# mmp/pbrt-v1

Measured on AMD Instinct MI355X. Metric: Mrays/s (primary+secondary: every Scene::Intersect + Scene::IntersectP), higher is better.
Workload: dtype f32

## Files before the change

### pbrt-v1_amd/csrc/hip/rt_device.h

```cpp
#pragma once
#include "rt_math.h"
#include "../../../include/pbrt_hip.h"
#include "../../../include/pbrt_hip_texture.h"

namespace rt {

struct DevTri { float4 q0, q1, q2; };
#define RT_PRIM_QUADRIC (1u << 17)
struct DevQuadric {
    float w2o[16], o2w[16];
    float radius, zmin, zmax, theta_min, theta_max, phi_max;
    int type, pad;
    float p1[3], p2[3], a, c;
};

#define RT_PRIM_SHADING (1u << 18)
#define RT_PRIM_TEXTURED (1u << 19)
struct DevTriShading {
    unsigned flags, xform;
    float uv[6];
    float dpdu[3];
    float n[9], s[9];
    float pad[3];
};

typedef RtMaterialResolved DevMaterial;
struct DevMatTex { RtMaterialParams raw; int textured; int prog_off[RT_MATSLOT_COUNT], prog_len[RT_MATSLOT_COUNT]; };

struct DevLight {
    int type;
    float color[3];
    float pos[3];
    int n_samples;
    unsigned first_tri, n_tris;
    int reverse_orientation, flip_normal;
    float area;
    float dir[3];
    int quadric;
    float w2l[9];
    float cos_total, cos_falloff;
};

#define RT_MAX_DIM_REQ 12
struct DimReq { unsigned f_base, u_base; unsigned short n; unsigned short dims; };

struct DevScene {
    const DevTri *tris;
    const DevQuadric *quadrics;
    const float4 *tri_shade;
    const uint2 *nodes;
    const uint2 *tnodes;
    const uint4 *tpairs;
    unsigned root_x, root_y;
    unsigned top_pairs, leaf_runs;
// ... 2 lines not shown
    const unsigned *leaf_refs;
    const int *tri_shading_idx;
    const DevTriShading *tri_shading;
    const float *xforms;
    const DevMaterial *materials;
    const DevLight *lights;
    const float *light_tris;
    unsigned n_tris, n_lights;
    float bounds[6];
    int accel_kind;
    int nvox[3];
    float gwidth[3], ginv_width[3];
    RtCamera cam;
    RtVolume vol;
    int dens_kind;
    float dens_a, dens_b, dens_up[3];
    int dens_n[3];
    const float *dens_grid;
    int n_infinite;
    int n_textured;
    const RtTexture *tex_nodes;
    const int *tex_prog;
    const DevMatTex *mat_tex;
    const int *tex_uv_idx;
    const float *tex_uv;
};

#define RT_INTEG_DIRECT_WEIGHTED 3

struct DevFrame {
    int integrator, max_depth, strategy, volume_integrator;
    float step_size;
    int sampler, xs, ys, jitter, spp;
    unsigned seed;
    int x_pixel_start, y_pixel_start, x_pixel_count, y_pixel_count;
    int x_start, x_end, y_start, y_end;
    float fxw, fyw, inv_fxw, inv_fyw;
    const float *filter_table;
    float *accum;
    float4 *samples;
    int shard_index, shard_count, tile_pixels;
    int tile_w, tile_h, tiles_x;
    int dbg_x, dbg_y;
    int exit_thresh;
    int phase_sync;
    int high_occupancy;
    int leaf_min;
    int mega_tile;
    int xcd_bands;
    int trav_mode;
    int pipeline;
    unsigned long long total_work;
    unsigned long long total_pixels;
    int n1d, n2d;
    unsigned lhs_total;
    unsigned pixgen_draws;
    DimReq one_d[RT_MAX_DIM_REQ];
    DimReq two_d[RT_MAX_DIM_REQ];
    const DimReq *light_dims;
    int dims_max_n;
    unsigned long long *work_counter;
    unsigned long long *counters;
    uint2 *spill;
    float *frames;
    float *vol_rays, *vol_state, *vol_samp;
    int vol_nmax;
    unsigned n_threads;
    int weighted_phase;
    unsigned *wt_base;
    float *wt_rec;
    float2 *wt_pick;
    int wt_mixed;
    unsigned wt_nd;
    const unsigned *wt_recbase;
    unsigned mat_pool_base;
    int dens_cap;
#ifdef RT_TAIL_PROBE
    unsigned long long *probe;
#endif
};

#if defined(__HIP_DEVICE_COMPILE__)
#define RT_G __attribute__((address_space(1)))
#define RT_L __attribute__((address_space(3)))
#else
#define RT_G
#define RT_L
#endif
typedef const DevMaterial RT_G &MatRef;
typedef const DevLight RT_G &LightRef;
#define RT_MAT(sc, i) (*((const DevMaterial RT_G *)(sc).materials + (i)))
#define RT_LIGHT(sc, i) (*((const DevLight RT_G *)(sc).lights + (i)))
#define RT_GPTR(T, p) ((T RT_G *)(p))

#define RT_SAMPLE_XY 1
__host__ __device__ inline unsigned long long sample_slot(unsigned lp, unsigned s, int spp) {
    return ((unsigned long long)(lp >> 6) * unsigned(spp) + s) * 128ull + (lp & 63u) * 2u;
}

}
```

### pbrt-v1_amd/csrc/hip/rt_integrate.h

```cpp
#pragma once
#include "rt_shade.h"
#include "rt_texture.h"

namespace rt {

enum Stage {
    ST_FETCH = 0, ST_VERTEX, ST_DIRECT_NEXT, ST_SHADOW_DONE, ST_MIS_DONE, ST_ED_BSDF, ST_ED_DONE,
    ST_BOUNCE, ST_SPECULAR, ST_SPEC_TRANS, ST_RETURN, ST_VOL_BEGIN, ST_VOL_STEP, ST_POP, ST_FINISH, ST_EXIT
};

struct Rng {
    uint32_t base, ctr;
    RT_DEV float next_float() { return rng_f32(base, ctr++); }
    RT_DEV uint32_t next_u32() { return rng_u32(base, ctr++); }
};

#define RT_FRAME_WORDS 25

struct Lane {
    uint32_t sample_index;
    uint32_t work;
    float image_x, image_y;
    uint32_t dim_base;
    Rng rng;
// ... 32 lines not shown
        if (pos == k) pos = other; else if (pos == other) pos = k;
    }
    float delta = 1.f / n;
    return (pos + rng_f32(ln.rng.base, fb + pos * r.dims + d)) * delta;
}

RT_DEV float van_der_corput(uint32_t n, uint32_t scramble) {
    n = (n << 16) | (n >> 16);
    n = ((n & 0x00ff00ffu) << 8) | ((n & 0xff00ff00u) >> 8);
    n = ((n & 0x0f0f0f0fu) << 4) | ((n & 0xf0f0f0f0u) >> 4);
    n = ((n & 0x33333333u) << 2) | ((n & 0xccccccccu) >> 2);
    n = ((n & 0x55555555u) << 1) | ((n & 0xaaaaaaaau) >> 1);
    n ^= scramble;
    return (float)n / (float)0x100000000LL;
}
RT_DEV float sobol2(uint32_t n, uint32_t scramble) {
    for (uint32_t v = 1u << 31; n != 0; n >>= 1, v ^= v >> 1)
        if (n & 0x1) scramble ^= v;
    return (float)scramble / (float)0x100000000LL;
}
RT_DEV int shuffle_origin(uint32_t base, uint32_t off, int count, int pos) {
    for (int k = count - 1; k >= 0; --k) {
        const int other = int(rng_u32(base, off + k) % uint32_t(count));
        if (pos == k) pos = other; else if (pos == other) pos = k;
    }
    return pos;
}
RT_DEV uint32_t pixel_stream(const DevFrame &fr, const Lane &ln) {
    const uint32_t n0 = ln.sample_index - (ln.work % uint32_t(fr.spp));
    if (n0 == 0 && fr.sampler != RT_SAMPLER_LOWDISCREPANCY) return rng_base(0xFFFFFFFFu, fr.seed);
    return rng_base(n0, fr.seed);
}
RT_DEV float dim_value(const DevFrame &fr, const Lane &ln, const DimReq &r, int j, int d) {
    if (fr.sampler == RT_SAMPLER_STRATIFIED) return lhs_value(ln, r, j, d);
    if (fr.sampler == RT_SAMPLER_RANDOM) return rng_f32(ln.rng.base, ln.dim_base + r.f_base + j * r.dims + d);
    const uint32_t pb = pixel_stream(fr, ln);
    const int P = fr.spp, n = r.n, s = int(ln.work % uint32_t(P));
    const uint32_t nscr = r.dims;
    const int blk = shuffle_origin(pb, r.f_base + nscr + uint32_t(n) * P, P, s);
    const int jb = (n == 1) ? 0 : shuffle_origin(pb, r.f_base + nscr + uint32_t(blk) * n, n, j);
    const uint32_t idx = uint32_t(blk) * n + jb;
    if (r.dims == 1) return van_der_corput(idx, rng_u32(pb, r.f_base));
    return d == 0 ? van_der_corput(idx, rng_u32(pb, r.f_base)) : sobol2(idx, rng_u32(pb, r.f_base + 1));
}

#ifndef RT_SAMPLE_NT
#define RT_SAMPLE_NT 1
#endif
RT_DEV void sample_write(const DevFrame &fr, const Lane &ln, V3 Ls, float alpha, unsigned &bad) {
    const float y = lum_y(Ls);
    if (Ls.x != Ls.x || Ls.y != Ls.y || Ls.z != Ls.z) { Ls = mk3(0.f); ++bad; }
    else if (y < -1e-5) { Ls = mk3(0.f); ++bad; }
    else if (isinf(y)) { Ls = mk3(0.f); ++bad; }
    const uint32_t lp = ln.work / uint32_t(fr.spp);
    float4 RT_G *rec = RT_GPTR(float4, fr.samples) + sample_slot(lp, ln.work - lp * uint32_t(fr.spp), fr.spp);
#if RT_SAMPLE_NT
    typedef float nt_f4 __attribute__((ext_vector_type(4)));
    const nt_f4 r0 = {Ls.x, Ls.y, Ls.z, alpha}, r1 = {ln.image_x, ln.image_y, 0.f, 0.f};
    __builtin_nontemporal_store(r0, (nt_f4 RT_G *)rec);
    __builtin_nontemporal_store(r1, (nt_f4 RT_G *)(rec + RT_SAMPLE_XY));
#else
    rec[0] = make_float4(Ls.x, Ls.y, Ls.z, alpha);
    rec[RT_SAMPLE_XY] = make_float4(ln.image_x, ln.image_y, 0.f, 0.f);
#endif
}

RT_DEV void stratified_camera_sample(const DevFrame &fr, uint32_t pixel_index, int s, int px, int py,
                                     uint32_t pix_base, float &ix, float &iy, float &lu, float &lv, bool need_lens) {
    const int n = fr.spp;
    const int sx = s % fr.xs, sy = s / fr.xs;
    const float dx = 1.f / fr.xs, dy = 1.f / fr.ys;
    float jx = 0.5f, jy = 0.5f;
    if (fr.jitter) { jx = rng_f32(pix_base, 2 * s); jy = rng_f32(pix_base, 2 * s + 1); }
    ix = (sx + jx) * dx; iy = (sy + jy) * dy;
    ix += px; iy += py;
    lu = lv = 0.5f;
    if (need_lens) {
        const uint32_t ub = fr.jitter ? 5u * n : 0u;
        int pos = s;
        for (int k = n - 1; k >= 0; --k) {
            int other = int(rng_u32(pix_base, ub + k) % uint32_t(n));
            if (pos == k) pos = other; else if (pos == other) pos = k;
        }
        const int lx = pos % fr.xs, ly = pos / fr.xs;
        float kx = 0.5f, ky = 0.5f;
        if (fr.jitter) { kx = rng_f32(pix_base, 2 * n + 2 * pos); ky = rng_f32(pix_base, 2 * n + 2 * pos + 1); }
        lu = (lx + kx) * dx; lv = (ly + ky) * dy;
    }
    (void)pixel_index;
}

RT_DEV Ray camera_ray(const RtCamera &cam, float ix, float iy, float lensU, float lensV) {
    Ray r;
    if (cam.type == RT_CAMERA_ENVIRONMENT) {
        r.o = xform_point(cam.camera_to_world, mk3(0.f, 0.f, 0.f));
        const float theta = RT_PI * iy / cam.y_res;
        const float phi = 2 * RT_PI * ix / cam.x_res;
        const V3 dir = mk3(sinf(theta) * cosf(phi), cosf(theta), sinf(theta) * sinf(phi));
        r.d = xform_vector(cam.camera_to_world, dir);
        r.mint = cam.hither; r.maxt = cam.yon;
        return r;
    }
    V3 Pcamera = xform_point(cam.raster_to_camera, mk3(ix, iy, 0.f));
    r.o = Pcamera;
    r.d = cam.type == RT_CAMERA_ORTHOGRAPHIC ? mk3(0.f, 0.f, 1.f) : Pcamera;
    if (cam.lens_radius > 0.f) {
        float lu, lv; concentric_disk(lensU, lensV, lu, lv);
        lu *= cam.lens_radius; lv *= cam.lens_radius;
        float ft = (cam.focal_distance - cam.hither) / r.d.z;
        V3 Pfocus = r.o + r.d * ft;
        r.o.x += lu * (cam.focal_distance - cam.hither) / cam.focal_distance;
        r.o.y += lv * (cam.focal_distance - cam.hither) / cam.focal_distance;
        r.d = Pfocus - r.o;
    }
    r.d = normalize3(r.d);
    r.mint = 0.f;
    r.maxt = cam.type == RT_CAMERA_ORTHOGRAPHIC ? cam.yon - cam.hither : (cam.yon - cam.hither) / r.d.z;
    r.o = xform_point(cam.camera_to_world, r.o);
    r.d = xform_vector(cam.camera_to_world, r.d);
    return r;
}

RT_DEV bool work_to_sample(const DevFrame &fr, unsigned long long w, unsigned long long &pixel, int &s) {
    const unsigned long long per_tile = (unsigned long long)fr.tile_pixels * fr.spp;
    if (fr.tile_w > 0) {
        const unsigned w32 = unsigned(w), pt = unsigned(per_tile);
        const unsigned lt = w32 / pt, rem = w32 - lt * pt;
        const unsigned tile = lt * unsigned(fr.shard_count) + unsigned(fr.shard_index);
        const unsigned q = rem / unsigned(fr.spp);
        s = int(rem - q * unsigned(fr.spp));
        const unsigned ty = tile / unsigned(fr.tiles_x), tx = tile - ty * unsigned(fr.tiles_x);
        const unsigned qy = q / unsigned(fr.tile_w), qx = q - qy * unsigned(fr.tile_w);
        const unsigned px = tx * unsigned(fr.tile_w) + qx, py = ty * unsigned(fr.tile_h) + qy;
        const unsigned ew = unsigned(fr.x_end - fr.x_start), eh = unsigned(fr.y_end - fr.y_start);
        pixel = (unsigned long long)py * ew + px;
        return px < ew && py < eh;
    }
    if (fr.total_work <= 0xffffffffull && per_tile <= 0xffffffffull) {
        const unsigned w32 = unsigned(w), pt = unsigned(per_tile);
        const unsigned lt = w32 / pt, rem = w32 - lt * pt;
        const unsigned long long tile = (unsigned long long)lt * unsigned(fr.shard_count) + unsigned(fr.shard_index);
        const unsigned q = rem / unsigned(fr.spp);
        pixel = tile * unsigned(fr.tile_pixels) + q;
        s = int(rem - q * unsigned(fr.spp));
        return pixel < fr.total_pixels;
    }
    const unsigned long long lt = w / per_tile, rem = w % per_tile;
    const unsigned long long tile = lt * fr.shard_count + fr.shard_index;
    pixel = tile * fr.tile_pixels + rem / fr.spp;
    s = int(rem % fr.spp);
    return pixel < fr.total_pixels;
}

RT_DEV void tile_order_to_sample(const DevFrame &fr, unsigned w, unsigned &pixel, int &s) {
    const unsigned spp = unsigned(fr.spp), T = unsigned(fr.mega_tile);
    const unsigned W = unsigned(fr.x_end - fr.x_start), H = unsigned(fr.y_end - fr.y_start);
    const unsigned wp = w / spp; s = int(w - wp * spp);
    const unsigned row_px = W * T, ty = wp / row_px, rem = wp - ty * row_px;
    const unsigned h_t = min(T, H - ty * T), full = T * h_t, tiles_x = (W + T - 1u) / T;
    unsigned tx = rem / full; tx = tx < tiles_x ? tx : tiles_x - 1u;
    const unsigned rem2 = rem - tx * full, w_t = min(T, W - tx * T);
    const unsigned qy = rem2 / w_t, qx = rem2 - qy * w_t;
    pixel = (ty * T + qy) * W + tx * T + qx;
}

RT_DEV void setup_sample(const DevScene &sc, const DevFrame &fr, Lane &ln, unsigned long long pixel, int s, Ray &ray) {
    const int w = fr.x_end - fr.x_start;
    int px, py;
    if (fr.total_pixels <= 0xffffffffull) { const unsigned row = unsigned(pixel) / unsigned(w); px = fr.x_start + int(unsigned(pixel) - row * unsigned(w)); py = fr.y_start + int(row); }
    else { px = fr.x_start + int(pixel % w); py = fr.y_start + int(pixel / w); }
    const uint32_t n0 = uint32_t(pixel * fr.spp);
    ln.sample_index = n0 + uint32_t(s);
    ln.rng.base = rng_base(ln.sample_index, fr.seed);
    float lu = 0.5f, lv = 0.5f;
    const bool need_lens = sc.cam.lens_radius > 0.f;
    if (fr.sampler == RT_SAMPLER_STRATIFIED) {
        const uint32_t pix_base = (pixel == 0) ? rng_base(0xFFFFFFFFu, fr.seed) : rng_base(n0, fr.seed);
        ln.dim_base = (s == 0 && pixel != 0) ? fr.pixgen_draws : 0u;
        stratified_camera_sample(fr, uint32_t(pixel), s, px, py, pix_base, ln.image_x, ln.image_y, lu, lv, need_lens);
    } else if (fr.sampler == RT_SAMPLER_RANDOM) {
        const uint32_t pix_base = (pixel == 0) ? rng_base(0xFFFFFFFFu, fr.seed) : rng_base(n0, fr.seed);
        ln.dim_base = (s == 0 && pixel != 0) ? fr.pixgen_draws : 0u;
        ln.image_x = rng_f32(pix_base, 2 * s); ln.image_y = rng_f32(pix_base, 2 * s + 1);
        ln.image_x += px; ln.image_y += py;
        if (need_lens) { lu = rng_f32(pix_base, 2 * fr.spp + 2 * s); lv = rng_f32(pix_base, 2 * fr.spp + 2 * s + 1); }
    } else {
        const uint32_t pix_base = rng_base(n0, fr.seed);
        const uint32_t P = uint32_t(fr.spp);
        ln.dim_base = (s == 0) ? fr.pixgen_draws : 0u;
        const int pos = shuffle_origin(pix_base, 2 + P, int(P), s);
        ln.image_x = px + van_der_corput(uint32_t(pos), rng_u32(pix_base, 0));
        ln.image_y = py + sobol2(uint32_t(pos), rng_u32(pix_base, 1));
        if (need_lens) {
            const uint32_t lb = 2 + 2 * P;
            const int lp = shuffle_origin(pix_base, lb + 2 + P, int(P), s);
            lu = van_der_corput(uint32_t(lp), rng_u32(pix_base, lb)); lv = sobol2(uint32_t(lp), rng_u32(pix_base, lb + 1));
        }
    }
    ln.rng.ctr = ln.dim_base + ((fr.sampler == RT_SAMPLER_LOWDISCREPANCY) ? 0u : fr.lhs_total);
    ray = camera_ray(sc.cam, ln.image_x, ln.image_y, lu, lv);
    ln.image_x = (ln.image_x + 1.f) - 1.f; ln.image_y = (ln.image_y + 1.f) - 1.f;
}

RT_DEV float RT_G *frame_ptr(const DevFrame &fr, int frame, unsigned gtid) {
    return RT_GPTR(float, fr.frames) + (size_t(frame) * RT_FRAME_WORDS) * fr.n_threads + gtid;
}
template <bool EXT>
RT_DEV void frame_push(const DevFrame &fr, Lane &ln, unsigned gtid, V3 f, float absdot, int after) {
    float RT_G *q = frame_ptr(fr, ln.fsp, gtid); const size_t st = fr.n_threads;
    q[0 * st] = ln.L.x; q[1 * st] = ln.L.y; q[2 * st] = ln.L.z;
    q[3 * st] = f.x; q[4 * st] = f.y; q[5 * st] = f.z; q[6 * st] = absdot;
    q[7 * st] = __int_as_float(after); q[8 * st] = __int_as_float(ln.depth);
    q[9 * st] = ln.v.p.x; q[10 * st] = ln.v.p.y; q[11 * st] = ln.v.p.z;
    q[12 * st] = ln.v.nn.x; q[13 * st] = ln.v.nn.y; q[14 * st] = ln.v.nn.z;
    q[15 * st] = ln.v.sn.x; q[16 * st] = ln.v.sn.y; q[17 * st] = ln.v.sn.z;
    q[18 * st] = ln.v.wo.x; q[19 * st] = ln.v.wo.y; q[20 * st] = ln.v.wo.z;
    q[21 * st] = __int_as_float(ln.v.mat);
    if (EXT) { q[22 * st] = ln.v.ng.x; q[23 * st] = ln.v.ng.y; q[24 * st] = ln.v.ng.z; }
    ++ln.fsp;
}
template <bool EXT>
RT_DEV int frame_pop(const DevFrame &fr, Lane &ln, unsigned gtid, V3 child) {
    --ln.fsp;
    const float RT_G *q = frame_ptr(fr, ln.fsp, gtid); const size_t st = fr.n_threads;
    V3 Lp = mk3(q[0 * st], q[1 * st], q[2 * st]);
    V3 f = mk3(q[3 * st], q[4 * st], q[5 * st]);
    float absdot = q[6 * st];
    ln.L = Lp + (child * f) * absdot;
    int after = __float_as_int(q[7 * st]);
    ln.depth = __float_as_int(q[8 * st]);
    ln.v.p = mk3(q[9 * st], q[10 * st], q[11 * st]);
    ln.v.nn = mk3(q[12 * st], q[13 * st], q[14 * st]);
    ln.v.sn = mk3(q[15 * st], q[16 * st], q[17 * st]);
    ln.v.tn = cross3(ln.v.nn, ln.v.sn);
    ln.v.wo = mk3(q[18 * st], q[19 * st], q[20 * st]);
    ln.v.mat = __float_as_int(q[21 * st]);
    if (EXT) ln.v.ng = mk3(q[22 * st], q[23 * st], q[24 * st]);
    return after;
}

template <bool DEFER = false>
RT_DEV void launch_ray(Lane &ln, const DevScene &sc, V3 o, V3 d, float mint, float maxt, bool any, int next_stage) {
    Ray r; r.o = o; r.d = d; r.mint = mint; r.maxt = maxt;
    if (DEFER) { ln.tv.o = o; ln.tv.d = d; ln.tv.mint = mint; ln.tv.maxt = maxt; ln.tv.any = any; ln.tv.hit_prim = -1; ln.tv.b1 = 0.f; ln.tv.b2 = 0.f; }
    else if (sc.accel_kind == RT_ACCEL_GRID) grid_begin(ln.tv, sc, r, any); else trav_begin(ln.tv, sc, r, any);
    ln.has_ray = true;
    ln.stage = next_stage;
}

RT_DEV float RT_G *vol_ray_ptr(const DevFrame &fr, int level, unsigned gtid) { return RT_GPTR(float, fr.vol_rays) + size_t(level) * 8 * fr.n_threads + gtid; }
RT_DEV void vol_store_ray(const DevFrame &fr, int level, unsigned gtid, const Ray &r) {
    float RT_G *q = vol_ray_ptr(fr, level, gtid); const size_t st = fr.n_threads;
    q[0] = r.o.x; q[st] = r.o.y; q[2 * st] = r.o.z; q[3 * st] = r.d.x; q[4 * st] = r.d.y; q[5 * st] = r.d.z; q[6 * st] = r.mint; q[7 * st] = r.maxt;
}
RT_DEV Ray vol_load_ray(const DevFrame &fr, int level, unsigned gtid) {
    const float RT_G *q = vol_ray_ptr(fr, level, gtid); const size_t st = fr.n_threads;
    Ray r; r.o = mk3(q[0], q[st], q[2 * st]); r.d = mk3(q[3 * st], q[4 * st], q[5 * st]); r.mint = q[6 * st]; r.maxt = q[7 * st];
    return r;
}
RT_DEV bool vol_intersect(const RtVolume &v, V3 o, V3 d, float mint, float maxt, float &t0, float &t1) {
    const V3 vo = xform_point(v.world_to_volume, o), vd = xform_vector(v.world_to_volume, d);
    float a = mint, b = maxt; bool ok = true;
#pragma unroll
    for (int i = 0; i < 3; ++i) {
        float invRayDir = 1.f / comp(vd, i);
        float tNear = (v.p0[i] - comp(vo, i)) * invRayDir, tFar = (v.p1[i] - comp(vo, i)) * invRayDir;
        if (tNear > tFar) { float tmp = tNear; tNear = tFar; tFar = tmp; }
        a = tNear > a ? tNear : a; b = tFar < b ? tFar : b;
        if (a > b) ok = false;
    }
    t0 = a; t1 = b; return ok;
}
RT_DEV bool vol_inside(const RtVolume &v, V3 p) {
    const V3 q = xform_point(v.world_to_volume, p);
    return q.x >= v.p0[0] && q.x <= v.p1[0] && q.y >= v.p0[1] && q.y <= v.p1[1] && q.z >= v.p0[2] && q.z <= v.p1[2];
}
RT_DEV V3 vol_transmittance(const RtVolume &v, V3 o, V3 d, float mint, float maxt) {
    float t0, t1;
    if (!vol_intersect(v, o, d, mint, maxt, t0, t1)) return mk3(1.f);
    const float dist = len3((o + d * t0) - (o + d * t1));
    const V3 tau = (mat_color(v.sigma_a) + mat_color(v.sigma_s)) * dist;
    return mk3(expf(-tau.x), expf(-tau.y), expf(-tau.z));
}
RT_DEV float lerp_ref(float t, float v1, float v2) { return (1.f - t) * v1 + t * v2; }
RT_DEV int clamp_ref(int v, int lo, int hi) { return v < lo ? lo : (v > hi ? hi : v); }
RT_DEV float density_at(const DevScene &sc, V3 q) {
    const RtVolume &v = sc.vol;
    if (!(q.x >= v.p0[0] && q.x <= v.p1[0] && q.y >= v.p0[1] && q.y <= v.p1[1] && q.z >= v.p0[2] && q.z <= v.p1[2])) return 0.f;
    if (sc.dens_kind == RT_DENSITY_EXPONENTIAL) {
        const float height = (q.x - v.p0[0]) * sc.dens_up[0] + (q.y - v.p0[1]) * sc.dens_up[1] + (q.z - v.p0[2]) * sc.dens_up[2];
        return sc.dens_a * expf(-sc.dens_b * height);
// ... 316 lines not shown
        return;
    }
    if constexpr (STAGE == ST_DIRECT_NEXT) {
        const int nLights = int(sc.n_lights);
        if constexpr (WEIGHTED) {
            if (nLights == 0) { ln.stage = ST_SPECULAR; return; }
            if (fr.weighted_phase == 1) { ++ln.ord; ln.stage = ST_SPECULAR; return; }
            if (fr.weighted_phase == 3 && ln.li > 0) { ln.stage = ST_SPECULAR; return; }
            if (fr.weighted_phase == 2 && fr.wt_mixed) {
                if (ln.li == 0 && ln.lj == 0) { ln.ctr0 = ln.rng.ctr; ln.wt_w = __uint_as_float(1u); }
                if (ln.li >= nLights) { ++ln.ord; ln.rng.ctr = ln.ctr0; ln.lj = 0; ln.stage = ST_SPECULAR; return; }
                ln.rng.ctr = ln.ctr0 + uint32_t(ln.lj);
            } else if (fr.weighted_phase == 2) {
                if (ln.li == 0) ln.ctr0 = ln.rng.ctr;
                if (ln.li >= nLights) { ++ln.ord; ln.stage = ST_SPECULAR; return; }
                ln.rng.ctr = ln.ctr0;
            }
            const float ls1 = dim_value(fr, ln, fr.two_d[0], 0, 0), ls2 = dim_value(fr, ln, fr.two_d[0], 0, 1);
            ln.bs1 = dim_value(fr, ln, fr.two_d[1], 0, 0); ln.bs2 = dim_value(fr, ln, fr.two_d[1], 0, 1);
            ln.bcs = dim_value(fr, ln, fr.one_d[1], 0, 0);
            if (fr.weighted_phase == 2) {
                if (ln.li == 0 && ln.lj == 0) RT_GPTR(float, fr.wt_rec)[weighted_record(fr, ln, nLights)] = dim_value(fr, ln, fr.one_d[0], 0, 0);
                estimate_direct_begin<EXT, DEFER>(sc, ln, ln.li, ls1, ls2);
            } else {
                const float2 pick = RT_GPTR(const float2, fr.wt_pick)[ln.ord++];
                ln.li = 1; ln.wt_w = pick.y;
                estimate_direct_begin<EXT, DEFER>(sc, ln, __float_as_int(pick.x), ls1, ls2);
            }
            return;
        }
        if (INTEG == RT_INTEGRATOR_PATH || (INTEG == RT_INTEGRATOR_DIRECT && fr.strategy == RT_STRATEGY_ONE)) {
            if (nLights == 0 || ln.li > 0) { ln.stage = (INTEG == RT_INTEGRATOR_PATH) ? ST_BOUNCE : ST_SPECULAR; return; }
            ln.li = 1;
            const int k = (INTEG == RT_INTEGRATOR_PATH) ? ln.depth : 0;
            const bool from_sampler = (INTEG == RT_INTEGRATOR_DIRECT) || k < 3;
            float un, ls1, ls2;
            if (from_sampler) {
                const int i1 = (INTEG == RT_INTEGRATOR_PATH) ? 3 * k : 0;
                const int i2 = (INTEG == RT_INTEGRATOR_PATH) ? 3 * k : 0;
                un = dim_value(fr, ln, fr.one_d[i1], 0, 0);
                ls1 = dim_value(fr, ln, fr.two_d[i2], 0, 0); ls2 = dim_value(fr, ln, fr.two_d[i2], 0, 1);
                ln.bs1 = dim_value(fr, ln, fr.two_d[i2 + 1], 0, 0); ln.bs2 = dim_value(fr, ln, fr.two_d[i2 + 1], 0, 1);
                ln.bcs = dim_value(fr, ln, fr.one_d[i1 + 1], 0, 0);
            } else {
                un = ln.rng.next_float();
                ls1 = ln.rng.next_float(); ls2 = ln.rng.next_float();
                ln.bs1 = ln.rng.next_float(); ln.bs2 = ln.rng.next_float(); ln.bcs = ln.rng.next_float();
            }
            int lightNum = min(int(floorf(un * nLights)), nLights - 1);
            estimate_direct_begin<EXT, DEFER>(sc, ln, lightNum, ls1, ls2);
            return;
        }
        if (INTEG == RT_INTEGRATOR_DIRECT) {
            if (ln.li >= nLights) { ln.L = ln.L + ln.L_all; ln.stage = ST_SPECULAR; return; }
            const DimReq RT_G *ld = RT_GPTR(const DimReq, fr.light_dims) + 3 * ln.li;
            const DimReq rl = ld[0], rb = ld[1], rc = ld[2];
            if (ln.lj == 0) ln.Ld_light = mk3(0.f);
            const float ls1 = dim_value(fr, ln, rl, ln.lj, 0), ls2 = dim_value(fr, ln, rl, ln.lj, 1);
            ln.bs1 = dim_value(fr, ln, rb, ln.lj, 0); ln.bs2 = dim_value(fr, ln, rb, ln.lj, 1);
            ln.bcs = dim_value(fr, ln, rc, ln.lj, 0);
            estimate_direct_begin<EXT, DEFER>(sc, ln, ln.li, ls1, ls2);
            return;
        }
        if (ln.li >= nLights) { ln.stage = ST_SPECULAR; return; }
        {
            LightRef Lt = RT_LIGHT(sc, ln.li);
            MatRef m = RT_MAT(sc, ln.v.mat);
            const int cur = ln.li++;
            V3 wi, Li, sd; float smax;
            if (light_is_delta<EXT>(Lt)) Li = delta_light_sample(Lt, ln.v.p, wi, sd, smax);
            else if constexpr (EXT) {
                if (light_is_infinite<EXT>(Lt)) {
                    float u2 = ln.rng.next_float();
                    float u1 = ln.rng.next_float();
                    float pdf; wi = infinite_sample_sphere(u1, u2, pdf);
                    Li = (pdf == 0.f) ? mk3(0.f) : div_s(mat_color(Lt.color), pdf);
                    sd = wi; smax = RT_INF;
                } else {
                    float u2 = ln.rng.next_float();
                    float u1 = ln.rng.next_float();
                    V3 ns; V3 ps = area_sample_point<EXT>(sc, Lt, ln.v.p, u1, u2, ln.rng, ns);
                    wi = normalize3(ps - ln.v.p);
                    float pdf = area_light_pdf<EXT>(sc, Lt, ln.v.p, wi);
                    Li = (pdf == 0.f) ? mk3(0.f) : div_s(area_L(Lt, ns, -wi), pdf);
                    sd = ps - ln.v.p; smax = 1.f - RT_RAY_EPSILON;
                }
            } else {
                float u2 = ln.rng.next_float();
                float u1 = ln.rng.next_float();
                V3 ns; V3 ps = area_sample_point<EXT>(sc, Lt, ln.v.p, u1, u2, ln.rng, ns);
                wi = normalize3(ps - ln.v.p);
                float pdf = area_light_pdf<EXT>(sc, Lt, ln.v.p, wi);
                Li = (pdf == 0.f) ? mk3(0.f) : div_s(area_L(Lt, ns, -wi), pdf);
                sd = ps - ln.v.p; smax = 1.f - RT_RAY_EPSILON;
            }
            (void)cur;
            if (is_black(Li)) return;
            V3 f = bsdf_f<EXT>(m, ln.v, ln.v.wo, wi);
            if (is_black(f)) return;
            ln.pend = (f * Li) * absdot3(wi, ln.v.nn);
            launch_ray<DEFER>(ln, sc, ln.v.p, sd, RT_RAY_EPSILON, smax, true, ST_SHADOW_DONE);
        }
        return;
    }
    if constexpr (STAGE == ST_SHADOW_DONE) {
        if (COUNT) ++*c_any;
        const bool occluded = ln.tv.hit_prim >= 0;
// ... 12 lines not shown
    }
    if constexpr (STAGE == ST_MIS_DONE) {
        if (COUNT) ++*c_closest;
        if (ln.tv.hit_prim >= 0) {
            V3 nh; int light;
            prim_normal_light<EXT>(sc, ln.tv, nh, light);
            if (light == ln.cur_light) {
                if (dot3(nh, -ln.tv.d) > 0)
                    ln.Ld = ln.Ld + ln.pend * scene_transmittance<VOL, EXT>(sc, fr, ln, ln.tv.o, ln.tv.d, ln.tv.mint, ln.tv.maxt);
            }
        } else if (EXT) {
            LightRef Lt = RT_LIGHT(sc, ln.cur_light);
            if (Lt.type == RT_LIGHT_INFINITE && !is_black(mat_color(Lt.color)))
                ln.Ld = ln.Ld + ln.pend * scene_transmittance<VOL, EXT>(sc, fr, ln, ln.tv.o, ln.tv.d, ln.tv.mint, ln.tv.maxt);
        }
        ln.stage = ST_ED_DONE;
        return;
    }
    if constexpr (STAGE == ST_ED_DONE) {
        const int nLights = int(sc.n_lights);
        if constexpr (WEIGHTED) {
            if (fr.weighted_phase == 2) {
                const unsigned at = fr.wt_mixed ? __float_as_uint(ln.wt_w) : 1u + 2u * unsigned(ln.li);
                float RT_G *rec = RT_GPTR(float, fr.wt_rec) + weighted_record(fr, ln, nLights) + at;
                rec[0] = lum_y(ln.Ld);
                rec[1] = lum_y(ln.Ld * float(nLights));
                if (fr.wt_mixed) {
                    ln.wt_w = __uint_as_float(at + 2u);
                    const unsigned j = ln.ord - RT_GPTR(const unsigned, fr.wt_base)[ln.work];
                    if (light_draws_rng(RT_LIGHT(sc, ln.li)) && unsigned(ln.lj) < j) ++ln.lj; else { ln.lj = 0; ++ln.li; }
                } else ++ln.li;
                ln.stage = ST_DIRECT_NEXT;
            } else {
                if (ln.wt_w == 0.f) ln.L = ln.L + ln.Ld * float(nLights);
                else ln.L = ln.L + div_s(ln.Ld, ln.wt_w);
                ln.stage = ST_SPECULAR;
            }
            return;
        }
        if (INTEG == RT_INTEGRATOR_PATH) {
            ln.L = ln.L + ln.thr * (ln.Ld * float(nLights));
            ln.stage = ST_BOUNCE;
        } else if (fr.strategy == RT_STRATEGY_ONE) {
            ln.L = ln.L + ln.Ld * float(nLights);
            ln.stage = ST_SPECULAR;
        } else {
            ln.Ld_light = ln.Ld_light + ln.Ld;
            const int ns = RT_GPTR(const DimReq, fr.light_dims)[3 * ln.li].n;
            if (++ln.lj >= ns) {
                ln.L_all = ln.L_all + ln.Ld_light * (1.f / float(ns));
                ln.lj = 0; ++ln.li;
            }
            ln.stage = ST_DIRECT_NEXT;
        }
        return;
    }
    if constexpr (STAGE == ST_BOUNCE) {
        MatRef m = RT_MAT(sc, ln.v.mat);
        const int k = ln.depth;
        float bs1, bs2, bcs;
        if (k < 3) {
            bs1 = dim_value(fr, ln, fr.two_d[3 * k + 2], 0, 0); bs2 = dim_value(fr, ln, fr.two_d[3 * k + 2], 0, 1);
            bcs = dim_value(fr, ln, fr.one_d[3 * k + 2], 0, 0);
        } else { bs1 = ln.rng.next_float(); bs2 = ln.rng.next_float(); bcs = ln.rng.next_float(); }
        V3 wi; float pdf; int flags;
        V3 f = bsdf_sample_f<EXT>(m, ln.v, ln.v.wo, wi, bs1, bs2, bcs, pdf, BX_ALL, flags);
        if (is_black(f) || pdf == 0.f) { ln.stage = ST_RETURN; return; }
        ln.specular = (flags & BX_SPECULAR) != 0;
        ln.thr = ln.thr * div_s(f * absdot3(wi, ln.v.nn), pdf);
        if (k > 3) {
            if (ln.rng.next_float() > .5f) { ln.stage = ST_RETURN; return; }
            ln.thr = div_s(ln.thr, .5f);
        }
        if (k == fr.max_depth) { ln.stage = ST_RETURN; return; }
        ++ln.depth;
        launch_ray<DEFER>(ln, sc, ln.v.p, wi, RT_RAY_EPSILON, RT_INF, false, ST_VERTEX);
        return;
    }
    if constexpr (STAGE == ST_SPECULAR) {
        if (!(ln.depth < fr.max_depth)) { ln.stage = ST_RETURN; return; }
        MatRef m = RT_MAT(sc, ln.v.mat);
        float u3 = ln.rng.next_float(), u2 = ln.rng.next_float(), u1 = ln.rng.next_float();
        V3 wi; float pdf; int flags;
        V3 f = bsdf_sample_f<EXT>(m, ln.v, ln.v.wo, wi, u1, u2, u3, pdf, BX_REFLECTION | BX_SPECULAR, flags);
        if (!is_black(f) && pdf > 0.f) f = div_s(f, pdf);
        const float ad = absdot3(wi, ln.v.nn);
        if (!is_black(f) && ad > 0.f) {
            frame_push<EXT>(fr, ln, gtid, f, ad, ST_SPEC_TRANS);
            ++ln.depth;
            launch_ray<DEFER>(ln, sc, ln.v.p, wi, RT_RAY_EPSILON, RT_INF, false, ST_VERTEX);
            if (VOL) { Ray cr; cr.o = ln.v.p; cr.d = wi; cr.mint = RT_RAY_EPSILON; cr.maxt = RT_INF; vol_store_ray(fr, ln.fsp, gtid, cr); }
            return;
        }
        ln.stage = ST_SPEC_TRANS;
        return;
    }
    if constexpr (STAGE == ST_SPEC_TRANS) {
        MatRef m = RT_MAT(sc, ln.v.mat);
        float u3 = ln.rng.next_float(), u2 = ln.rng.next_float(), u1 = ln.rng.next_float();
        V3 wi; float pdf; int flags;
        V3 f = bsdf_sample_f<EXT>(m, ln.v, ln.v.wo, wi, u1, u2, u3, pdf, BX_TRANSMISSION | BX_SPECULAR, flags);
        if (!is_black(f) && pdf > 0.f) f = div_s(f, pdf);
        const float ad = absdot3(wi, ln.v.nn);
        if (!is_black(f) && ad > 0.f) {
            frame_push<EXT>(fr, ln, gtid, f, ad, ST_RETURN);
            ++ln.depth;
// ... 172 lines not shown
```

### pbrt-v1_amd/csrc/hip/rt_kernels.hip

```cpp
#include "rt_host.h"
#include "rt_weighted.h"

namespace rt {
__global__ void camera_kernel(DevScene sc, DevFrame fr, unsigned long long first, unsigned count, RtRay *out) {
    const unsigned i = blockIdx.x * blockDim.x + threadIdx.x;
    if (i >= count) return;
    const unsigned long long n = first + i;
    Lane ln; Ray r;
    setup_sample(sc, fr, ln, n / fr.spp, int(n % fr.spp), r);
    out[i].o[0] = r.o.x; out[i].o[1] = r.o.y; out[i].o[2] = r.o.z;
    out[i].d[0] = r.d.x; out[i].d[1] = r.d.y; out[i].d[2] = r.d.z;
    out[i].mint = r.mint; out[i].maxt = r.maxt;
}

}

namespace rt {
const char *knob(const char *name) {
#ifdef RT_NO_TUNABLES
    (void)name; return nullptr;
#else
    static const bool on = std::getenv("PBRT_HIP_TUNE") != nullptr;
    return on ? std::getenv(name) : nullptr;
#endif
// ... 403 lines not shown
            HIPCHK(hipMemcpy(s->light_dims, up.data(), up.size() * sizeof(DimReq), hipMemcpyHostToDevice));
        }
        fr.light_dims = s->light_dims;
        d1.erase(d1.begin(), d1.begin() + (all_lights ? nl : 4 * RT_BD_MAX_VERTS + 1));
        d2.clear();
    }
    if (d1.size() > RT_MAX_DIM_REQ || d2.size() > RT_MAX_DIM_REQ) return fail(RT_ESTATE, "rt_render: sample table overflow");
    fr.n1d = int(d1.size()); fr.n2d = int(d2.size());
    std::memset(fr.one_d, 0, sizeof fr.one_d); std::memset(fr.two_d, 0, sizeof fr.two_d);
    for (size_t i = 0; i < d1.size(); ++i) fr.one_d[i] = d1[i];
    for (size_t i = 0; i < d2.size(); ++i) fr.two_d[i] = d2[i];
    {
        const size_t nn = s->tree.nodes.size();
        if (s->per_leaf < 0.0) {
            size_t leaves = 0, refs = 0;
            if (s->accel_kind == RT_ACCEL_KDTREE) for (const Node &n : s->tree.nodes) if ((n.x & 3u) == 3u && (n.x >> 2)) { ++leaves; refs += n.x >> 2; }
            s->per_leaf = leaves ? double(refs) / double(leaves) : 1.0;
        }
        const double per_leaf = s->per_leaf;
        const bool tiny = nn <= 4096 && per_leaf >= 1.5;
        const bool tiny_path = tiny && rd->integrator == RT_INTEGRATOR_PATH;
        fr.trav_mode = (tiny && !tiny_path) ? 3 : 2;
        fr.exit_thresh = tiny ? (rd->integrator == RT_INTEGRATOR_PATH ? 8 : 0) : 32;
        if (RT_MEGA_BYV && tiny && rd->integrator == RT_INTEGRATOR_PATH && !s->volume.present && !s->has_ext) fr.exit_thresh = 16;
        fr.high_occupancy = (tiny && !tiny_path) ? 0 : 1;
        if (const char *e = knob("PBRT_HIP_HIGH_OCC")) fr.high_occupancy = std::atoi(e);
        fr.leaf_min = tiny ? 8 : RT_TRACE_LEAF_MIN;
        if (const char *e = knob("PBRT_HIP_LEAF_MIN")) fr.leaf_min = std::max(1, std::atoi(e));
        if (const char *e = knob("PBRT_HIP_TRAV_MODE")) fr.trav_mode = std::atoi(e);
        fr.xcd_bands = rd->integrator != RT_INTEGRATOR_PATH ? 1 : 0;
        if (const char *e = knob("PBRT_HIP_XCD_BANDS")) fr.xcd_bands = std::atoi(e) != 0;
        if (const char *e = knob("PBRT_HIP_EXIT_THRESH")) fr.exit_thresh = std::atoi(e);
        fr.dbg_x = fr.dbg_y = -1000000;
        if (const char *e = knob("PBRT_HIP_DEBUG_PIXEL")) std::sscanf(e, "%d,%d", &fr.dbg_x, &fr.dbg_y);
        fr.phase_sync = tiny ? 1 : 0;
        if (const char *e = knob("PBRT_HIP_PHASE_SYNC")) fr.phase_sync = std::atoi(e);
        fr.pipeline = (!tiny && s->volume.present) ? 1 : 0;
        if (const char *e = knob("PBRT_HIP_PIPELINE")) fr.pipeline = std::atoi(e) != 0;
        if (fr.max_depth > 250 || fr.max_depth < 0) fr.pipeline = 0;
        if (fr.dims_max_n >= 65535) fr.pipeline = 0;
        if (s->dev.n_lights >= 65535u) fr.pipeline = 0;
        if (rd->integrator == RT_INTEGRATOR_DIRECT && rd->strategy == RT_STRATEGY_WEIGHTED) fr.pipeline = 0;
        if (bidir) { fr.pipeline = 0; fr.xcd_bands = 0; }
        if (rd->integrator == RT_INTEGRATOR_DEBUG) { fr.pipeline = 0; fr.high_occupancy = 0; }
        if (fr.shard_count == 1 && !fr.pipeline) {
            fr.tile_w = fr.tile_h = fr.tiles_x = 0; fr.tile_pixels = 1;
            fr.total_work = fr.total_pixels * fr.spp;
            fr.mega_tile = 32;
            if (const char *e = knob("PBRT_HIP_MEGA_TILE")) fr.mega_tile = std::max(0, std::atoi(e));
            if (fr.mega_tile > 4096 || fr.total_work > 0xffffffffull) fr.mega_tile = 0;
        }
        if (fr.trav_mode != 3 || fr.high_occupancy) fr.trav_mode = 2;
    }
    fr.work_counter = s->work_counter; fr.counters = s->counters; fr.spill = s->spill; fr.n_threads = s->n_threads;
    fr.frames = s->frames;
    if (need_film && !s->accum) return fail(RT_ESTATE, "rt_render: no film bound (call rt_film_bind first)");
    if (need_film && (fr.x_pixel_count != s->film_w || fr.y_pixel_count != s->film_h))
        return fail(RT_EINVAL, "rt_render: film size does not match the bound film");
    return RT_OK;
}

int rt_camera_rays(RtScene *s, const RtRenderDesc *rd, uint64_t first, uint32_t count, RtRay *rays_out) {
    if (!s || !rd || !rays_out) return fail(RT_EINVAL, "null argument");
    HIPCHK(hipSetDevice(s->device));
    DevFrame fr; int rc = make_frame(s, rd, fr, false); if (rc) return rc;
    DevBuf<RtRay> dev;
    if ((rc = dev.grow(count ? count : 1))) return rc;
    hipLaunchKernelGGL(camera_kernel, dim3((count + 255) / 256), dim3(256), 0, s->stream, s->dev, fr,
                       (unsigned long long)first, count, dev.p);
    HIPCHK(hipGetLastError());
    HIPCHK(hipStreamSynchronize(s->stream));
    HIPCHK(hipMemcpy(rays_out, dev, size_t(count) * sizeof(RtRay), hipMemcpyDeviceToHost));
    return RT_OK;
}

static int trace_common(RtScene *s, const RtRay *rays, uint32_t n, int any, RtHit *hits, uint8_t *occ) {
    if (!s || !rays || (!hits && !occ)) return fail(RT_EINVAL, "null argument");
    HIPCHK(hipSetDevice(s->device));
    if (n == 0) return RT_OK;
    if (int rc = ensure(s, s->trace_buf, size_t(n) * 3)) return rc;
    std::vector<float4> host(size_t(n) * 2);
    for (uint32_t i = 0; i < n; ++i) {
        host[i] = make_float4(rays[i].o[0], rays[i].o[1], rays[i].o[2], rays[i].mint);
        host[size_t(n) + i] = make_float4(rays[i].d[0], rays[i].d[1], rays[i].d[2], rays[i].maxt);
    }
    unsigned qc[RT_QC_STRIDE] = {0};
    qc[0] = any ? 0u : n; qc[RT_QC_ANY] = any ? n : 0u;
    HIPCHK(hipMemcpyAsync(s->trace_buf, host.data(), host.size() * sizeof(float4), hipMemcpyHostToDevice, s->stream));
    HIPCHK(hipMemcpyAsync(s->trace_qc, qc, sizeof qc, hipMemcpyHostToDevice, s->stream));
    TraceJob job{};
    job.q_o = s->trace_buf; job.q_d = s->trace_buf + n; job.q_slot = nullptr; job.q_count = s->trace_qc; job.hit = s->trace_buf + 2 * size_t(n);
    job.n_slots = 0; job.spill = s->spill; job.n_threads = s->n_threads; job.counters = s->counters;
    flavour::Request rq = request_of(s);
    rq.count = true;
    const int k = flavour::Trace::index(rq);
    HIPWARN(hipEventRecord(s->ev0, s->stream));
    hipLaunchKernelGGL(g_pipe_trace[k], dim3(s->grids.trace[k]), dim3(RT_BLOCK), 0, s->stream, (const DevScene *)s->dev_scene, job);
    HIPWARN(hipEventRecord(s->ev1, s->stream)); HIPWARN(hipEventRecord(s->ev2, s->stream)); s->have_timing = true; s->last_pipeline = false;
    HIPCHK(hipGetLastError());
    HIPCHK(hipMemcpyAsync(host.data(), s->trace_buf + 2 * size_t(n), size_t(n) * sizeof(float4), hipMemcpyDeviceToHost, s->stream));
    HIPCHK(hipStreamSynchronize(s->stream));
    for (uint32_t i = 0; i < n; ++i) {
        int prim; std::memcpy(&prim, &host[i].x, 4);
        if (any) occ[i] = prim >= 0 ? 1 : 0;
        else { hits[i].prim = prim; hits[i].t = host[i].y; hits[i].b1 = host[i].z; hits[i].b2 = host[i].w; }
    }
// ... 184 lines not shown
```

Measured before the change: 3417.

## Replace runtime integer divisions with precomputed magic-number fast division

Precomputes multiply-shift reciprocals for spp, strata width, image width, tile and mega-tile sizes on the host and stores them in the frame. Device-side sample indexing and pixel mapping then use mulhi plus shifts instead of slow 32-bit integer division. It also ends direct lighting in the same step once the last light finishes, saving one stage dispatch per vertex. The frame struct grows, which adds kernel-argument size.

```diff
diff --git a/pbrt-v1_amd/csrc/hip/rt_device.h b/pbrt-v1_amd/csrc/hip/rt_device.h
--- a/pbrt-v1_amd/csrc/hip/rt_device.h
+++ b/pbrt-v1_amd/csrc/hip/rt_device.h
@@ -1,5 +1,6 @@
 #pragma once
 #include "rt_math.h"
+#include "rt_fastdiv.h"
 #include "../../../include/pbrt_hip.h"
 #include "../../../include/pbrt_hip_texture.h"
 
@@ -108,6 +109,7 @@
     int pipeline;
     unsigned long long total_work;
     unsigned long long total_pixels;
+    FrameDiv div;
     int n1d, n2d;
     unsigned lhs_total;
     unsigned pixgen_draws;
diff --git a/pbrt-v1_amd/csrc/hip/rt_fastdiv.h b/pbrt-v1_amd/csrc/hip/rt_fastdiv.h
--- /dev/null
+++ b/pbrt-v1_amd/csrc/hip/rt_fastdiv.h
@@ -0,0 +1,67 @@
+#pragma once
+#include <cstdint>
+
+#if defined(__HIPCC__) || defined(__CUDACC__)
+#define RT_FASTDIV_FN __host__ __device__ inline
+#else
+#define RT_FASTDIV_FN inline
+#endif
+
+namespace rt {
+
+struct FastDiv {
+    uint32_t mul, sh1, sh2;
+};
+
+inline FastDiv fastdiv_make(uint32_t d) {
+    FastDiv f = {0u, 0u, 0u};
+    if (d == 0u) return f;
+    uint32_t l = 0;
+    while (l < 32u && (uint64_t(1) << l) < d) ++l;
+    f.mul = uint32_t(((uint64_t(1) << 32) * ((uint64_t(1) << l) - d)) / d + 1u);
+    f.sh1 = l < 1u ? l : 1u;
+    f.sh2 = l > 0u ? l - 1u : 0u;
+    return f;
+}
+
+RT_FASTDIV_FN uint32_t fastdiv_mulhi(uint32_t a, uint32_t b) {
+#if defined(__HIP_DEVICE_COMPILE__)
+    return __umulhi(a, b);
+#else
+    return uint32_t((uint64_t(a) * uint64_t(b)) >> 32);
+#endif
+}
+
+RT_FASTDIV_FN uint32_t fastdiv(uint32_t n, const FastDiv &f) {
+    const uint32_t t = fastdiv_mulhi(f.mul, n);
+    return (t + ((n - t) >> f.sh1)) >> f.sh2;
+}
+
+struct FrameDiv {
+    FastDiv spp;
+    FastDiv xs;
+    FastDiv width;
+    FastDiv row_px;
+    FastDiv block[2];
+    FastDiv block_w[2];
+    uint32_t blocks_x;
+    FastDiv per_tile;
+    FastDiv tile_w, tiles_x;
+};
+
+inline FrameDiv framediv_make(uint32_t spp, uint32_t xs, uint32_t W, uint32_t H, uint32_t T, uint64_t per_tile, uint32_t tile_w, uint32_t tiles_x) {
+    FrameDiv fd = {};
+    fd.spp = fastdiv_make(spp); fd.xs = fastdiv_make(xs); fd.width = fastdiv_make(W);
+    if (T > 0u && uint64_t(W) * T <= 0xffffffffull) {
+        const uint32_t h_last = H - (H - 1u) / T * T, w_last = W - (W - 1u) / T * T;
+        fd.row_px = fastdiv_make(W * T);
+        fd.block[0] = fastdiv_make(T * T); fd.block[1] = fastdiv_make(T * h_last);
+        fd.block_w[0] = fastdiv_make(T); fd.block_w[1] = fastdiv_make(w_last);
+        fd.blocks_x = (W - 1u) / T + 1u;
+    }
+    if (per_tile <= 0xffffffffull) fd.per_tile = fastdiv_make(uint32_t(per_tile));
+    fd.tile_w = fastdiv_make(tile_w); fd.tiles_x = fastdiv_make(tiles_x);
+    return fd;
+}
+
+}
diff --git a/pbrt-v1_amd/csrc/hip/rt_integrate.h b/pbrt-v1_amd/csrc/hip/rt_integrate.h
--- a/pbrt-v1_amd/csrc/hip/rt_integrate.h
+++ b/pbrt-v1_amd/csrc/hip/rt_integrate.h
@@ -108,7 +108,7 @@
     if (Ls.x != Ls.x || Ls.y != Ls.y || Ls.z != Ls.z) { Ls = mk3(0.f); ++bad; }
     else if (y < -1e-5) { Ls = mk3(0.f); ++bad; }
     else if (isinf(y)) { Ls = mk3(0.f); ++bad; }
-    const uint32_t lp = ln.work / uint32_t(fr.spp);
+    const uint32_t lp = fastdiv(ln.work, fr.div.spp);
     float4 RT_G *rec = RT_GPTR(float4, fr.samples) + sample_slot(lp, ln.work - lp * uint32_t(fr.spp), fr.spp);
 #if RT_SAMPLE_NT
     typedef float nt_f4 __attribute__((ext_vector_type(4)));
@@ -124,7 +124,7 @@
 RT_DEV void stratified_camera_sample(const DevFrame &fr, uint32_t pixel_index, int s, int px, int py,
                                      uint32_t pix_base, float &ix, float &iy, float &lu, float &lv, bool need_lens) {
     const int n = fr.spp;
-    const int sx = s % fr.xs, sy = s / fr.xs;
+    const int sy = int(fastdiv(unsigned(s), fr.div.xs)), sx = s - sy * fr.xs;
     const float dx = 1.f / fr.xs, dy = 1.f / fr.ys;
     float jx = 0.5f, jy = 0.5f;
     if (fr.jitter) { jx = rng_f32(pix_base, 2 * s); jy = rng_f32(pix_base, 2 * s + 1); }
@@ -181,12 +181,12 @@
     const unsigned long long per_tile = (unsigned long long)fr.tile_pixels * fr.spp;
     if (fr.tile_w > 0) {
         const unsigned w32 = unsigned(w), pt = unsigned(per_tile);
-        const unsigned lt = w32 / pt, rem = w32 - lt * pt;
+        const unsigned lt = fastdiv(w32, fr.div.per_tile), rem = w32 - lt * pt;
         const unsigned tile = lt * unsigned(fr.shard_count) + unsigned(fr.shard_index);
-        const unsigned q = rem / unsigned(fr.spp);
+        const unsigned q = fastdiv(rem, fr.div.spp);
         s = int(rem - q * unsigned(fr.spp));
-        const unsigned ty = tile / unsigned(fr.tiles_x), tx = tile - ty * unsigned(fr.tiles_x);
-        const unsigned qy = q / unsigned(fr.tile_w), qx = q - qy * unsigned(fr.tile_w);
+        const unsigned ty = fastdiv(tile, fr.div.tiles_x), tx = tile - ty * unsigned(fr.tiles_x);
+        const unsigned qy = fastdiv(q, fr.div.tile_w), qx = q - qy * unsigned(fr.tile_w);
         const unsigned px = tx * unsigned(fr.tile_w) + qx, py = ty * unsigned(fr.tile_h) + qy;
         const unsigned ew = unsigned(fr.x_end - fr.x_start), eh = unsigned(fr.y_end - fr.y_start);
         pixel = (unsigned long long)py * ew + px;
@@ -194,9 +194,9 @@
     }
     if (fr.total_work <= 0xffffffffull && per_tile <= 0xffffffffull) {
         const unsigned w32 = unsigned(w), pt = unsigned(per_tile);
-        const unsigned lt = w32 / pt, rem = w32 - lt * pt;
+        const unsigned lt = fastdiv(w32, fr.div.per_tile), rem = w32 - lt * pt;
         const unsigned long long tile = (unsigned long long)lt * unsigned(fr.shard_count) + unsigned(fr.shard_index);
-        const unsigned q = rem / unsigned(fr.spp);
+        const unsigned q = fastdiv(rem, fr.div.spp);
         pixel = tile * unsigned(fr.tile_pixels) + q;
         s = int(rem - q * unsigned(fr.spp));
         return pixel < fr.total_pixels;
@@ -211,19 +211,22 @@
 RT_DEV void tile_order_to_sample(const DevFrame &fr, unsigned w, unsigned &pixel, int &s) {
     const unsigned spp = unsigned(fr.spp), T = unsigned(fr.mega_tile);
     const unsigned W = unsigned(fr.x_end - fr.x_start), H = unsigned(fr.y_end - fr.y_start);
-    const unsigned wp = w / spp; s = int(w - wp * spp);
-    const unsigned row_px = W * T, ty = wp / row_px, rem = wp - ty * row_px;
-    const unsigned h_t = min(T, H - ty * T), full = T * h_t, tiles_x = (W + T - 1u) / T;
-    unsigned tx = rem / full; tx = tx < tiles_x ? tx : tiles_x - 1u;
+    const FrameDiv &dv = fr.div;
+    const unsigned wp = fastdiv(w, dv.spp); s = int(w - wp * spp);
+    const unsigned row_px = W * T, ty = fastdiv(wp, dv.row_px), rem = wp - ty * row_px;
+    const unsigned h_t = min(T, H - ty * T), full = T * h_t, tiles_x = dv.blocks_x;
+    const FastDiv &df = h_t < T ? dv.block[1] : dv.block[0];
+    unsigned tx = fastdiv(rem, df); tx = tx < tiles_x ? tx : tiles_x - 1u;
     const unsigned rem2 = rem - tx * full, w_t = min(T, W - tx * T);
-    const unsigned qy = rem2 / w_t, qx = rem2 - qy * w_t;
+    const FastDiv &dw = w_t < T ? dv.block_w[1] : dv.block_w[0];
+    const unsigned qy = fastdiv(rem2, dw), qx = rem2 - qy * w_t;
     pixel = (ty * T + qy) * W + tx * T + qx;
 }
 
 RT_DEV void setup_sample(const DevScene &sc, const DevFrame &fr, Lane &ln, unsigned long long pixel, int s, Ray &ray) {
     const int w = fr.x_end - fr.x_start;
     int px, py;
-    if (fr.total_pixels <= 0xffffffffull) { const unsigned row = unsigned(pixel) / unsigned(w); px = fr.x_start + int(unsigned(pixel) - row * unsigned(w)); py = fr.y_start + int(row); }
+    if (fr.total_pixels <= 0xffffffffull) { const unsigned row = fastdiv(unsigned(pixel), fr.div.width); px = fr.x_start + int(unsigned(pixel) - row * unsigned(w)); py = fr.y_start + int(row); }
     else { px = fr.x_start + int(pixel % w); py = fr.y_start + int(pixel / w); }
     const uint32_t n0 = uint32_t(pixel * fr.spp);
     ln.sample_index = n0 + uint32_t(s);
@@ -293,6 +296,11 @@
     ln.v.mat = __float_as_int(q[21 * st]);
     if (EXT) ln.v.ng = mk3(q[22 * st], q[23 * st], q[24 * st]);
     return after;
+}
+
+RT_DEV void all_lights_done(Lane &ln) {
+    ln.L = ln.L + ln.L_all;
+    ln.stage = ST_SPECULAR;
 }
 
 template <bool DEFER = false>
@@ -715,7 +723,7 @@
             return;
         }
         if (INTEG == RT_INTEGRATOR_DIRECT) {
-            if (ln.li >= nLights) { ln.L = ln.L + ln.L_all; ln.stage = ST_SPECULAR; return; }
+            if (ln.li >= nLights) { all_lights_done(ln); return; }
             const DimReq RT_G *ld = RT_GPTR(const DimReq, fr.light_dims) + 3 * ln.li;
             const DimReq rl = ld[0], rb = ld[1], rc = ld[2];
             if (ln.lj == 0) ln.Ld_light = mk3(0.f);
@@ -834,6 +842,7 @@
                 ln.lj = 0; ++ln.li;
             }
             ln.stage = ST_DIRECT_NEXT;
+            if (ln.li >= nLights) all_lights_done(ln);
         }
         return;
     }
diff --git a/pbrt-v1_amd/csrc/hip/rt_kernels.hip b/pbrt-v1_amd/csrc/hip/rt_kernels.hip
--- a/pbrt-v1_amd/csrc/hip/rt_kernels.hip
+++ b/pbrt-v1_amd/csrc/hip/rt_kernels.hip
@@ -479,6 +479,8 @@
         }
         if (fr.trav_mode != 3 || fr.high_occupancy) fr.trav_mode = 2;
     }
+    fr.div = framediv_make(unsigned(fr.spp), unsigned(fr.xs), unsigned(fr.x_end - fr.x_start), unsigned(fr.y_end - fr.y_start), unsigned(fr.mega_tile),
+                           (unsigned long long)fr.tile_pixels * fr.spp, unsigned(fr.tile_w), unsigned(fr.tiles_x));
     fr.work_counter = s->work_counter; fr.counters = s->counters; fr.spill = s->spill; fr.n_threads = s->n_threads;
     fr.frames = s->frames;
     if (need_film && !s->accum) return fail(RT_ESTATE, "rt_render: no film bound (call rt_film_bind first)");
```

Measured after the change: 3495 (median of 6 runs). 2.3% higher.
